# tud-amr/semantic_dsp_map

Measured on AMD Instinct MI355X. Metric: Mvoxels updated/sec (256^3 grid, 2M particles, VKITTI2 camera; whole hot-path frame), higher is better.
Workload: dtype f32

## Files before the change

### semantic_dsp_map_amd/csrc/kernels.hip

```cpp
#include <algorithm>

#include <type_traits>

#include <hip/hip_ext.h>
#include "sdm_internal.h"
#include "sdm_scratch.h"

#pragma clang fp contract(off)

namespace sdm {

namespace {

constexpr int TPB = 256;

#ifdef SDM_AB_TIMERS
}
__device__ unsigned long long g_dbg[6][8192 * 4];
namespace {
#define DBG_T() wall_clock64()
#define DBG_PUTK(k, i, v) do { if (blockIdx.x < 8192) g_dbg[k][blockIdx.x * 4 + (i)] = (unsigned long long)(v); } while (0)
#define DBG_PUT(i, v) DBG_PUTK(0, i, v)
#define DBG_LANE0(k, i) do { if (threadIdx.x == 0 && threadIdx.y == 0) DBG_PUTK(k, i, DBG_T()); } while (0)
#else
// ... 1497 lines not shown
      continue;
    }
    if (camz[i] > dpt * d.occl_coeff) continue;
    observed = true;
    vis[i] = true;
  }
  const uint32_t sub = (shard + (threadIdx.x & 63u)) & (ROW_SUBS - 1);
  uint32_t rq[S];
#pragma unroll
  for (int i = 1; i < S; ++i)
    if (vis[i]) {
      pib[i] = atomicAdd(&sc.bin_count[pixv[i]], 1u);
      rq[i] = atomicAdd(&sc.row_cnt[(size_t)(rowv[i] * ROW_SUBS + sub) * ROW_CNT_STRIDE], 1u);
    }
#pragma unroll
  for (int i = 1; i < S; ++i)
    if (vis[i]) {
      if (rq[i] < sc.row_cap && pib[i] < (1u << ROW_PIB_BITS)) {
        const uint32_t col = (uint32_t)(pixv[i] - rowv[i] * d.W);
        sc.row_list[(size_t)(rowv[i] * ROW_SUBS + sub) * sc.row_cap + rq[i]] =
            make_uint2((uint32_t)(((size_t)v << d.p_n) + i), col | pib[i] << ROW_COL_BITS);
      } else {
        sc.cnt->overflow = 1;
      }
    }
  if (dirty) rec_store_status<S>(rec, stv);
  if (dirty || wrote_free) st.vflag[lv] = VF_DIRTY;
  bool stamped = observed;
  if (!observed && valid_n == 0) stamped = im_ok && im_z <= im_depth;
  if (stamped) st.vts[lv] = (uint16_t)f.gts;
  if (dirty || wrote_free || stamped) mark_tile(st, lv, f.epoch);
}

constexpr int VIS_WORDS = 32;
constexpr int VIS_J = VIS_WORDS * 64 / TPB;

template <int S>
__global__ __launch_bounds__(TPB) void k_visibility(Dims d, State st, Scratch sc) {
  __shared__ unsigned long long wmask[VIS_WORDS];
  __shared__ uint32_t woff[VIS_WORDS + 1];
  __shared__ uint16_t full_list[VIS_WORDS * 64];
  __shared__ uint32_t n_full;
  DBG_LANE0(1, 0);
  const Frame f = sc.fa->f;
  const gptr<float> depth_img = as_global(sc.fa->depth);
  const uint32_t fgen = (uint32_t)sc.fa->force_generic, fcx = (uint32_t)sc.cnt->flood_complex;
  const bool generic = (fgen | fcx) != 0;
  if (blockIdx.x == 0 && threadIdx.x == 0) {
    sc.cnt->vis_flood_complex = fcx;
    sc.cnt->vis_flood_rounds = sc.cnt->flood_rounds;
    sc.cnt->vis_start_in_frustum = sc.cnt->start_in_frustum;
  }
  const int bx = f.bb1[0] - f.bb0[0], by = f.bb1[1] - f.bb0[1], bz = f.bb1[2] - f.bb0[2];
  if (bx <= 0 || by <= 0 || bz <= 0) return;
  const int wlo = f.bb0[0] >> 6, nwx = ((f.bb1[0] - 1) >> 6) - wlo + 1;
  const uint32_t n_words = (uint32_t)nwx * by * bz;
  for (uint32_t g0 = blockIdx.x * VIS_WORDS; g0 < n_words; g0 += gridDim.x * VIS_WORDS) {
  __syncthreads();
  if (threadIdx.x == 0) n_full = 0;
  if (threadIdx.x < VIS_WORDS) {
    const uint32_t g = g0 + threadIdx.x;
    unsigned long long m = 0;
    if (g < n_words) {
      const int wi = wlo + (int)(g % nwx);
      const int ay = f.bb0[1] + (int)((g / nwx) % by);
      const int az = f.bb0[2] + (int)(g / ((uint32_t)nwx * by));
      const uint32_t rz = axis_correct(az + f.eq[2], d.NZ);
      if (rz >= d.rz_begin && rz < d.rz_begin + d.rz_count) {
        const uint64_t *__restrict__ bits = generic ? sc.reach : sc.vmask;
        const int VY = d.NY + 1;
        unsigned long long w0[4], w1[4], lr[4];
        const int wi1 = wi + 1 < (int)sc.wpl ? wi + 1 : wi;
#pragma unroll
        for (int c = 0; c < 4; ++c) {
          const int y = ay + (c & 1), z = az + (c >> 1);
          const size_t lb = ((size_t)z * VY + y) * sc.wpl;
          lr[c] = sc.line_reach[(size_t)z * sc.wy + (y >> 6)];
          w0[c] = bits[lb + wi];
          w1[c] = bits[lb + wi1];
        }
        __builtin_amdgcn_sched_barrier(0);
#pragma unroll
        for (int c = 0; c < 4; ++c) {
          const int y = ay + (c & 1);
          const bool line_ok = generic || ((lr[c] >> (y & 63)) & 1ull);
          const unsigned long long w1m = wi + 1 < (int)sc.wpl ? w1[c] : 0ull;
          if (line_ok) m |= w0[c] | (w0[c] >> 1) | (w1m << 63);
        }
        const int x0 = wi << 6;
        const int lo = f.bb0[0] > x0 ? f.bb0[0] - x0 : 0;
        const int hi = f.bb1[0] - x0 < 64 ? f.bb1[0] - x0 : 64;
// ... 91 lines not shown
}

__device__ __forceinline__ void sift_down(uint32_t *a, uint32_t start, uint32_t end) {
  uint32_t root = start;
  while (2 * root + 1 <= end) {
    uint32_t child = 2 * root + 1, sw = root;
    if (a[sw] < a[child]) sw = child;
    if (child + 1 <= end && a[sw] < a[child + 1]) sw = child + 1;
    if (sw == root) return;
    uint32_t t = a[root];
    a[root] = a[sw];
    a[sw] = t;
    root = sw;
  }
}

constexpr int A7_ROWS = 16;
constexpr int A7_ITEMS = 16;
constexpr uint32_t CK_LIGHT_MAX = 4;
enum : uint8_t { CK_DONE = 0, CK_LIGHT = 1, CK_HEAVY = 2 };

__device__ __forceinline__ void ck_store(const Filter &flt, const Scratch &sc, float *__restrict__ ck_out, int finish, int p,
                                         const sdm_labeled_point &o, float ck) {
  if (finish) {
    const float ckk = ck * flt.p_detect + flt.noise_number;
    sc.ck_kappa[p] = ckk;
    sc.pix4[p] = make_float4(o.x, o.y, o.z, ckk);
    sc.pixt[p] = (uint32_t)o.track_id | (1u << 16);
  } else {
    ck_out[p] = ck;
  }
}

constexpr int BR_TPB = 640;
constexpr int BR_WAVES = BR_TPB / 64;
constexpr int BR_MAXW = 1 << ROW_COL_BITS;
template <int PPT>
__global__ __launch_bounds__(BR_TPB) __attribute__((amdgpu_waves_per_eu(PPT <= 4 ? 5 : 4, PPT <= 4 ? 5 : 4))) void k_bin_rows(Dims d, State st, Scratch sc) {
  static_assert(PPT == 2 || PPT == 4 || PPT * BR_TPB >= BR_MAXW, "eight pixels per thread cover the widest image");
  __shared__ uint32_t pre[BR_MAXW + 1];
  __shared__ uint32_t wave_tot[BR_WAVES];
  __shared__ uint32_t s_base;
  const int r = blockIdx.x;
  DBG_LANE0(2, 0);
  if (r == (int)gridDim.x - 1 && threadIdx.x < 64) alias_compact_wave(st);
  const bool overflow = sc.cnt->overflow != 0;
  const int lane = threadIdx.x & 63, wid = threadIdx.x >> 6;
  const int W = d.W;
  uint32_t c[PPT];
  const int j0 = PPT * (int)threadIdx.x;
#pragma unroll
  for (int u = 0; u < PPT; ++u) c[u] = (!overflow && j0 + u < W) ? sc.bin_count[r * W + j0 + u] : 0u;
  uint32_t sub_n = 0;
  if (threadIdx.x < ROW_SUBS && !overflow) {
    sub_n = sc.row_cnt[(size_t)(r * ROW_SUBS + threadIdx.x) * ROW_CNT_STRIDE];
    if (sub_n > sc.row_cap) sub_n = sc.row_cap;
  }
  uint32_t inc = 0;
#pragma unroll
  for (int u = 0; u < PPT; ++u) inc += c[u];
  const uint32_t mine = inc;
#pragma unroll
  for (int off = 1; off < 64; off <<= 1) {
    const uint32_t t = __shfl_up(inc, off, 64);
    if (lane >= off) inc += t;
  }
  if (lane == 63) wave_tot[wid] = inc;
  __syncthreads();
  uint32_t before = 0, total = 0;
#pragma unroll
  for (int w = 0; w < BR_WAVES; ++w) {
    if (w < wid) before += wave_tot[w];
    total += wave_tot[w];
  }
  {
    uint32_t run = before + inc - mine;
#pragma unroll
    for (int u = 0; u < PPT; ++u) {
      if (j0 + u < W) pre[j0 + u] = run;
      run += c[u];
    }
  }
  if (threadIdx.x == 0) {
    pre[W] = total;
    s_base = total ? atomicAdd(&sc.cnt->n_vis, total) : 0u;
    if (total && (s_base > sc.cap_vis || total > sc.cap_vis - s_base)) {
      sc.cnt->overflow = 1;
      pre[W] = 0;
    }
  }
  uint32_t sub_ex[ROW_SUBS + 1];
  {
    uint32_t run = 0;
#pragma unroll
    for (int k = 0; k < ROW_SUBS; ++k) {
      sub_ex[k] = run;
      run += (uint32_t)__shfl(sub_n, k, 64);
    }
    sub_ex[ROW_SUBS] = run;
  }
  __shared__ uint32_t s_sub[ROW_SUBS + 1];
  if (threadIdx.x == 0) {
#pragma unroll
    for (int k = 0; k <= ROW_SUBS; ++k) s_sub[k] = sub_ex[k];
  }
  __syncthreads();
  const uint32_t base = s_base;
  uint32_t *__restrict__ bs = sc.bin_start + (size_t)r * (W + 1);
  const bool row_over = total != 0 && pre[W] == 0;
  {
    const int h = d.window_half;
#pragma unroll
    for (int u = 0; u < PPT; ++u) {
      const int j = j0 + u;
      if (j < W) {
        const uint32_t n = row_over ? 0u : pre[j + h + 1 > W ? W : j + h + 1] - pre[j - h < 0 ? 0 : j - h];
        sc.row_win[r * W + j] = (uint8_t)(n > 255u ? 255u : n);
      }
    }
  }
  for (int j = threadIdx.x; j <= W; j += BR_TPB) bs[j] = row_over ? 0u : base + pre[j];
  if (total == 0 || row_over) {
    DBG_LANE0(2, 1);
    return;
  }
  const uint32_t n_row = s_sub[ROW_SUBS];
  for (uint32_t g = threadIdx.x; g < n_row; g += BR_TPB) {
    int sub = 0;
#pragma unroll
    for (int k = 1; k < ROW_SUBS; ++k) sub += s_sub[k] <= g ? 1 : 0;
    const uint2 e = sc.row_list[(size_t)(r * ROW_SUBS + sub) * sc.row_cap + (g - s_sub[sub])];
    sc.bin_idx[base + pre[e.y & (uint32_t)(BR_MAXW - 1)] + (e.y >> ROW_COL_BITS)] = e.x;
  }
  __syncthreads();
  const size_t slot_base = (size_t)d.v_begin << d.p_n;
#pragma unroll
  for (int u = 0; u < PPT; ++u) {
    const uint32_t n = c[u];
    if (!n) continue;
    const uint32_t p = (uint32_t)(r * W + j0 + u);
    const uint32_t s = base + pre[j0 + u];
    uint32_t *a = sc.bin_idx + s;
    auto small_bin = [&](auto kk) {
      constexpr int K = decltype(kk)::value;
      uint32_t v[K];
#pragma unroll
      for (int i = 0; i < K; ++i) v[i] = (uint32_t)i < n ? a[i] : 0xffffffffu;
#pragma unroll
      for (int pass = 0; pass < K; ++pass)
#pragma unroll
        for (int i = pass & 1; i + 1 < K; i += 2) {
          const uint32_t lo = v[i] < v[i + 1] ? v[i] : v[i + 1], hi = v[i] < v[i + 1] ? v[i + 1] : v[i];
          v[i] = lo;
// ... 36 lines not shown
    if (n > 1) {
      if (n <= 32) {
        for (uint32_t i = 1; i < n; ++i) {
          uint32_t x = a[i];
          uint32_t j = i;
          while (j > 0 && a[j - 1] > x) {
            a[j] = a[j - 1];
            --j;
          }
          a[j] = x;
        }
      } else {
        for (int start = (int)(n - 2) / 2; start >= 0; --start) sift_down(a, (uint32_t)start, n - 1);
        for (uint32_t end = n - 1; end > 0; --end) {
          uint32_t t = a[end];
          a[end] = a[0];
          a[0] = t;
          sift_down(a, 0, end - 1);
        }
      }
    }
    for (uint32_t i = 0; i < n; ++i) {
      const size_t li = (size_t)a[i] - slot_base;
      const float4 q = st.pos4[li];
      const SlotRef sr = slot_ref_li(st, d.p_n, li);
      sc.vp4[s + i] = make_float4(q.x, q.y, q.z, sr.w());
      sc.vtf[s + i] = (uint32_t)sr.track() | ((uint32_t)st.forget[li] << 16);
      sc.vpix[s + i] = p;
    }
  }
  DBG_LANE0(2, 1);
}

__global__ __launch_bounds__(TPB) void k_ck_classify(Dims d, Filter flt, Scratch sc, float *__restrict__ ck_out, int finish) {
  const uint32_t p = blockIdx.x * blockDim.x + threadIdx.x;
  const int W = d.W, H = d.H, h = d.window_half;
  const bool in_image = p < (uint32_t)(W * H);
  const bool overflow = sc.cnt->overflow != 0;
  sdm_labeled_point o;
  o.is_valid = 0;
  uint32_t total = 0;
  if (in_image) {
    o = load_point(sc.fa->cloud, p);
    const int i = (int)p / W;
    uint32_t rw[A7_ROWS];
#pragma unroll
    for (int r = 0; r < A7_ROWS; ++r) {
      const int ni = i + r - h;
      const bool ok = r <= 2 * h && ni >= 0 && ni < H;
      rw[r] = sc.row_win[(int)p + (ok ? (r - h) * W : 0)];
    }
    __builtin_amdgcn_sched_barrier(0);
#pragma unroll
    for (int r = 0; r < A7_ROWS; ++r) {
      const int ni = i + r - h;
      total += (r <= 2 * h && ni >= 0 && ni < H) ? rw[r] : 0u;
    }
  }
  uint8_t cls = CK_DONE;
  if (in_image && o.is_valid && total != 0 && !overflow) cls = total <= CK_LIGHT_MAX ? CK_LIGHT : CK_HEAVY;
  const unsigned long long hm = __ballot(cls == CK_HEAVY);
  if (hm) {
    const uint32_t lane = threadIdx.x & 63u;
    const uint32_t shard = blockIdx.x & (VIS_SHARDS - 1);
    uint32_t base = 0;
    if (lane == 0) base = atomicAdd(&sc.cnt->shard[shard].heavy, (uint32_t)__popcll(hm));
    base = (uint32_t)__shfl((int)base, 0, 64);
    if (cls == CK_HEAVY) sc.ck_heavy[shard * sc.cap_heavy + base + (uint32_t)__popcll(hm & ((1ull << lane) - 1ull))] = p;
  }
  if (!in_image) return;
  if (!finish) {
    sc.pix4[p] = make_float4(o.x, o.y, o.z, 0.f);
    sc.pixt[p] = o.is_valid ? ((uint32_t)o.track_id | (1u << 16)) : 0u;
  }
  if (!o.is_valid) {
    if (finish) sc.pixt[p] = 0;
  } else if (cls == CK_DONE) {
    ck_store(flt, sc, ck_out, finish, (int)p, o, 0.f);
  }
  sc.ck_class[p] = cls;
}


template <bool FAST>
__device__ __forceinline__ float ck_term(const Filter &flt, const float *__restrict__ pdf, const float4 pv, const uint32_t tf,
                                         const sdm_labeled_point &o, float rsig, bool &skip) {
  const uint16_t ptrack = (uint16_t)(tf & 0xffffu);
  skip = flt.independent && ptrack != o.track_id;
  const float fg = flt.forget[(tf >> 16) & 7];
  float gk = query_pdf_r<FAST>(pdf, pv.x, o.x, o.sigma, rsig) * query_pdf_r<FAST>(pdf, pv.y, o.y, o.sigma, rsig) *
             query_pdf_r<FAST>(pdf, pv.z, o.z, o.sigma, rsig);
  if (!flt.independent) {
    gk *= fg;
    if (ptrack != o.track_id) gk *= flt.id_transition;
  }
  return pv.w * gk;
}

__device__ __forceinline__ void ck_light_pixel(const Dims &d, const Filter &flt, const State &st, const Scratch &sc,
                                               float *__restrict__ ck_out, int finish, int p) {
  const bool mine = p < d.W * d.H && sc.ck_class[p] == CK_LIGHT;
  sdm_labeled_point o;
  uint32_t ss[A7_ROWS], ee[A7_ROWS];
  if (mine) {
    o = load_point(sc.fa->cloud, p);
    const int h = d.window_half;
    const int i = p / d.W, j = p - i * d.W;
    const int j0 = j - h < 0 ? 0 : j - h;
    const int j1 = j + h >= d.W ? d.W - 1 : j + h;
#pragma unroll
    for (int r = 0; r < A7_ROWS; ++r) {
      const int ni = i + r - h;
      ss[r] = ee[r] = 0;
      if (r <= 2 * h && ni >= 0 && ni < d.H) {
        ss[r] = sc.bin_start[ni * (d.W + 1) + j0];
// ... 30 lines not shown
#endif
constexpr uint32_t CK_TERM_CAP = SDM_CK_TERM_CAP;

#ifndef SDM_CK_HEAVY_PER_LIST
#define SDM_CK_HEAVY_PER_LIST 28
#endif
constexpr uint32_t CK_HEAVY_BLOCKS = SDM_CK_HEAVY_PER_LIST * VIS_SHARDS;
#ifndef SDM_CK_WAVES
#define SDM_CK_WAVES 7
#endif
#define CK_WAVES_ATTR __attribute__((amdgpu_waves_per_eu(SDM_CK_WAVES, SDM_CK_WAVES)))

__global__ __launch_bounds__(A7_ROWS *A7_ITEMS) CK_WAVES_ATTR void k_ck(Dims d, Filter flt, State st, Scratch sc,
                                                          float *__restrict__ ck_out, int finish) {
  DBG_LANE0(3, 0);
  if (blockIdx.x >= CK_HEAVY_BLOCKS) {
    ck_light_pixel(d, flt, st, sc, ck_out, finish,
                   (int)((blockIdx.x - CK_HEAVY_BLOCKS) * (A7_ROWS * A7_ITEMS) + threadIdx.y * A7_ROWS + threadIdx.x));
    DBG_LANE0(3, 1);
    return;
  }
  __shared__ float rowsum[A7_ITEMS][A7_ROWS];
  __shared__ uint32_t rowoff[A7_ITEMS * A7_ROWS + 1];
  __shared__ uint32_t rowbeg[A7_ITEMS * A7_ROWS];
  __shared__ float opx[A7_ITEMS][5];
  __shared__ uint32_t otrk[A7_ITEMS];
  __shared__ float term[CK_TERM_CAP];
  __shared__ uint8_t rowof[CK_TERM_CAP];
  const int r = threadIdx.x, it = threadIdx.y;
  const int lane = it * A7_ROWS + r;
  const int h = d.window_half;
  const uint32_t shard = blockIdx.x & (VIS_SHARDS - 1);
  const uint32_t n = sc.cnt->shard[shard].heavy;
  const float *__restrict__ pdf = st.pdf;
  const gptr<sdm_labeled_point> cloud_img = as_global(sc.fa->cloud);
  __shared__ uint32_t s_q0, s_slow;
  for (;;) {
    __syncthreads();
    if (lane == 0) {
      s_q0 = atomicAdd(&sc.cnt->shard[shard].heavy_ticket, (uint32_t)A7_ITEMS);
      s_slow = 0;
    }
    __syncthreads();
    const uint32_t q0 = s_q0;
    if (q0 >= n) break;
#ifdef SDM_AB_TIMERS
    if (lane == 0) g_dbg[3][blockIdx.x * 4 + 2] += 1;
#endif
    const uint32_t q = q0 + it;
    int p = 0;
    uint32_t s = 0, e = 0;
    sdm_labeled_point o;
    if (q < n) {
      p = (int)sc.ck_heavy[shard * sc.cap_heavy + q];
      o = load_point(sc.fa->cloud, p);
      const int i = p / d.W, j = p - i * d.W;
      const int ni = i + r - h;
      if (r <= 2 * h && ni >= 0 && ni < d.H) {
        const int j0 = j - h < 0 ? 0 : j - h;
        const int j1 = j + h >= d.W ? d.W - 1 : j + h;
        s = sc.bin_start[ni * (d.W + 1) + j0];
        e = sc.bin_start[ni * (d.W + 1) + j1 + 1];
      }
      if (r == 0) {
        opx[it][0] = o.x;
        opx[it][1] = o.y;
// ... 1159 lines not shown
    const uint32_t seg = n_tiles <= TPB * OCC_SEG_MAX ? ((n_tiles + TPB - 1) / TPB + 15u) / 16u * 16u : 0u;
    if (seg) grid = dim3(std::min<uint32_t>(OCC_GRID, n_tiles));
    SDM_DISPATCH_S(k_occupancy, grid, s, d, flt.occ_threshold, st, cnt, fa, n_tiles, seg);
  }
}


void launch_set_frame(FrameArgs *fa_dev, const FrameArgs &fa, hipStream_t s) {
  hipLaunchKernelGGL(k_set_frame, dim3(1), dim3(TPB), 0, s, fa_dev, fa);
}
const void *set_frame_kernel() { return reinterpret_cast<const void *>(k_set_frame); }

void launch_frustum(const Dims &d, const Scratch &sc, hipStream_t s) {
  static bool lds_attr_set = false;
  if (!lds_attr_set) {
    (void)hipFuncSetAttribute(reinterpret_cast<const void *>(k_flood2d), hipFuncAttributeMaxDynamicSharedMemorySize, 152 * 1024);
    lds_attr_set = true;
  }
  const size_t max_words = (size_t)(d.NY + 1) * (d.NZ + 1) * sc.wpl;
  const unsigned g_mask = (unsigned)std::min<size_t>(blocks_for(max_words * 64), 4096);
  const unsigned g_line = (unsigned)std::min<size_t>(blocks_for((size_t)sc.wy * (d.NZ + 1) * 64), 256);
  hipLaunchKernelGGL(k_vertex_mask, dim3(g_mask), dim3(TPB), 0, s, d, sc.fa_side, sc.vmask, sc.wpl, sc.cnt);
  hipLaunchKernelGGL(k_line_info, dim3(g_line), dim3(TPB), 0, s, d, sc.fa_side, sc.vmask, sc.wpl, sc.wy, sc.line_ne, sc.line_ey, sc.line_ez,
                     sc.cnt);
  hipLaunchKernelGGL(k_flood2d, dim3(1), dim3(TPB), (size_t)(d.NZ + 1) * sc.wy * 8 * 4, s, d, sc.fa_side, sc.vmask, sc.wpl, sc.wy, sc.line_ey,
                     sc.line_ez, sc.line_reach, sc.cnt);
  hipLaunchKernelGGL(k_flood_generic, dim3(1), dim3(1024), 0, s, d, sc.fa_side, sc.vmask, sc.reach, sc.wpl, sc.cnt);
}

void launch_visibility(const Dims &d, const Filter &flt, const State &st, const Scratch &sc, float *ck_out, int finish, hipStream_t s,
                       hipEvent_t vis_done) {
  {
    const size_t max_words = (size_t)((d.NX + 63) / 64 + 1) * d.NY * d.NZ;
    dim3 grid((unsigned)std::min<size_t>(blocks_for(max_words, VIS_WORDS), 2048));
    if (vis_done) {
      switch (d.p_n) {
        case 1: hipExtLaunchKernelGGL(k_visibility<2>, grid, dim3(TPB), 0, s, nullptr, vis_done, 0, d, st, sc); break;
        case 2: hipExtLaunchKernelGGL(k_visibility<4>, grid, dim3(TPB), 0, s, nullptr, vis_done, 0, d, st, sc); break;
        case 3: hipExtLaunchKernelGGL(k_visibility<8>, grid, dim3(TPB), 0, s, nullptr, vis_done, 0, d, st, sc); break;
        default: hipExtLaunchKernelGGL(k_visibility<16>, grid, dim3(TPB), 0, s, nullptr, vis_done, 0, d, st, sc); break;
      }
    } else {
      SDM_DISPATCH_S(k_visibility, grid, s, d, st, sc);
    }
  }
  if (d.W <= 2 * BR_TPB) hipLaunchKernelGGL(k_bin_rows<2>, dim3((unsigned)d.H), dim3(BR_TPB), 0, s, d, st, sc);
  else if (d.W <= 4 * BR_TPB) hipLaunchKernelGGL(k_bin_rows<4>, dim3((unsigned)d.H), dim3(BR_TPB), 0, s, d, st, sc);
  else hipLaunchKernelGGL(k_bin_rows<8>, dim3((unsigned)d.H), dim3(BR_TPB), 0, s, d, st, sc);
  hipLaunchKernelGGL(k_ck_classify, dim3(blocks_for((size_t)d.W * d.H)), dim3(TPB), 0, s, d, flt, sc, ck_out, finish);
}

void launch_ck(const Dims &d, const Filter &flt, const State &st, const Scratch &sc, float *ck_out, int finish, hipStream_t s) {
  hipLaunchKernelGGL(k_ck, dim3(CK_HEAVY_BLOCKS + blocks_for((size_t)d.W * d.H, A7_ROWS * A7_ITEMS)), dim3(A7_ROWS, A7_ITEMS), 0, s, d, flt, st, sc,
                     ck_out, finish);
}
void launch_ck_finish(const Dims &d, const Filter &flt, const Scratch &sc, const float *parts, int n_parts, size_t part_stride, hipStream_t s) {
  hipLaunchKernelGGL(k_ck_finish, dim3(blocks_for((size_t)d.W * d.H)), dim3(TPB), 0, s, d, flt, sc, parts, n_parts,
                     part_stride ? part_stride : (size_t)d.W * d.H);
}
void launch_ck_reduce_chunk(const float *stage, const float *own_part, float *full, uint32_t chunk, int world, int rank, hipStream_t s) {
  hipLaunchKernelGGL(k_ck_reduce_chunk, dim3((chunk + TPB - 1) / TPB), dim3(TPB), 0, s, stage, own_part, full, chunk, world, rank);
}
void launch_weight(const Dims &d, const Filter &flt, const State &st, const Scratch &sc, hipStream_t s, const float *ck_raw) {
  const int side = 2 * d.window_half + 1;
#define SDM_WEIGHT(UU, RR)                                                                                              \
  if (ck_raw) hipLaunchKernelGGL((k_weight<UU, RR, true>), dim3(WT_GRID), dim3(64 * WT_WAVES), 0, s, d, flt, st, sc, ck_raw); \
  else hipLaunchKernelGGL((k_weight<UU, RR, false>), dim3(WT_GRID), dim3(64 * WT_WAVES), 0, s, d, flt, st, sc, ck_raw);
  if (side * side <= 64) {
    SDM_WEIGHT(4, 1)
  } else if (side * side <= 128) {
    SDM_WEIGHT(4, 2)
  } else {
    SDM_WEIGHT(2, 4)
  }
#undef SDM_WEIGHT
}

int launch_birth_prepare(const Dims &d, const Filter &flt, const BirthOrder &bo, const State &st,
                         const Scratch &sc, hipStream_t s) {
  const size_t hw = (size_t)d.W * d.H;
  const size_t total = hw * flt.nb;
  if (flt.use_rng) {
// ... 189 lines not shown
```

### semantic_dsp_map_amd/csrc/lifecycle.hip

```cpp
#include <rocrand/rocrand.h>

#include <chrono>
#include <cmath>
#include <cstdlib>
#include <mutex>

#include "sdm_map.h"

#pragma clang fp contract(off)

namespace {

thread_local std::string g_last_error;

__attribute__((constructor(101))) void sdm_runtime_defaults() {
  setenv("HIP_FORCE_DEV_KERNARG", "1", 0);
}

constexpr double GRAPH_PIECES_US = 110.0, GRAPH_CHAIN_US = 170.0;
constexpr int LAUNCHES_PER_FRAME = 50;

__global__ void k_noop() {}

}
// ... 410 lines not shown
  A(m->st.alias, 2 + 2 * ALIAS_CAP);
  m->st.alias_cap = ALIAS_CAP;
  HIP_TRY(hipMemsetAsync(m->st.alias, 0, 8, m->stream));
  A(m->st.alias_filter, ALIAS_FILTER_WORDS);
  HIP_TRY(hipMemsetAsync(m->st.alias_filter, 0, ALIAS_FILTER_WORDS * 4, m->stream));
  A(m->st.res, d.v_count);
  A(m->st.stamps_x, d.NX);
  A(m->st.stamps_y, d.NY);
  A(m->st.stamps_z, d.NZ);
  A(m->st.pdf, PDF_NUM);
  m->noise_n = 1000000;
  A(m->st.noise, m->noise_n);
  HIP_TRY(hipMemsetAsync(m->st.noise, 0, (size_t)m->noise_n * 4, m->stream));
  {
    std::vector<float> pdf;
    build_pdf_table(pdf);
    HIP_TRY(hipMemcpyAsync(m->st.pdf, pdf.data(), PDF_NUM * 4, hipMemcpyHostToDevice, m->stream));
    HIP_TRY(hipStreamSynchronize(m->stream));
  }
  Scratch &sc = m->sc;
  sc.wpl = (int)((d.NX + 1 + 63) / 64);
  const size_t n_words = (size_t)(d.NZ + 1) * (d.NY + 1) * sc.wpl;
  A(sc.vmask, n_words);
  A(sc.reach, n_words);
  sc.wy = (int)((d.NY + 1 + 63) / 64);
  const size_t n_line_words = (size_t)(d.NZ + 1) * sc.wy;
  A(sc.line_ne, n_line_words);
  A(sc.line_ey, n_line_words);
  A(sc.line_ez, n_line_words);
  A(sc.line_reach, n_line_words);
  A(m->d_depth, hw);
  A(m->d_cloud, hw);
  A(sc.bin_count, hw + 1 + (size_t)d.H * ROW_SUBS * ROW_CNT_STRIDE);
  A(sc.row_win, hw);
  sc.row_cnt = sc.bin_count + hw + 1;
  A(sc.bin_start, (size_t)d.H * (d.W + 1));
  size_t cap_vis = cfg->max_visible > 0 ? (size_t)cfg->max_visible
                                        : std::min<size_t>(n_slots + (size_t)VIS_SHARDS * 256 * d.S, (size_t)16 << 20);
  cap_vis = (cap_vis + VIS_SHARDS - 1) / VIS_SHARDS * VIS_SHARDS;
  cap_vis = std::min<size_t>(cap_vis, 0xffffff00u);
  sc.cap_vis = (uint32_t)cap_vis;
  {
    const size_t row_total = std::min<size_t>(cap_vis, std::max<size_t>(2 * cap_vis / (size_t)d.H, (size_t)2 * d.W * d.S));
    sc.row_cap = (uint32_t)std::max<size_t>(64, (row_total + row_total / 4) / ROW_SUBS + 64);
  }
  A(sc.row_list, (size_t)d.H * ROW_SUBS * sc.row_cap);
  A(sc.bin_idx, cap_vis);
  A(sc.vpix, cap_vis);
  A(sc.vp4, cap_vis);
  A(sc.vtf, cap_vis);
  A(sc.pix4, hw);
  A(sc.pixt, hw);
  A(sc.ck_kappa, hw);
  sc.cap_heavy = (uint32_t)(((hw + 255) / 256 + VIS_SHARDS - 1) / VIS_SHARDS * 256);
  A(sc.ck_heavy, (size_t)sc.cap_heavy * VIS_SHARDS);
  A(sc.ck_class, hw);
  m->ck_chunk = (uint32_t)(((hw + shard_count - 1) / shard_count + 63) / 64 * 64);
  A(m->d_ck_part, (size_t)m->ck_chunk * shard_count);
  for (auto &r : m->raw) {
    A(r.depth, hw);
    A(r.static_mask, hw);
    A(r.label_to_inst, 256);
    A(r.bbox, 6 * MAX_CLOUD_OBJECTS);
  }
  A(sc.b_valid, hw + 1);
  A(sc.b_rank, hw + 1);
  sc.cap_move = (uint32_t)std::min<size_t>((size_t)d.V * d.S, (size_t)1 << 18);
  A(m->d_counts_local, HALO_OBJ);
  const size_t mv_cnt_n = move_count_elems();
  A(sc.mv_cnt, mv_cnt_n);
  A(sc.mv_list, 8192);
  A(sc.mv_nlist, 4);
  HIP_TRY(hipMemsetAsync(sc.mv_nlist, 0, 4 * sizeof(uint32_t), m->stream));
  A(sc.mv_nmem, 8192);
  A(sc.mv_mem, move_member_elems(n_slots));
  A(sc.mv_tot, move_total_elems());
  HIP_TRY(hipMemsetAsync(sc.mv_tot, 0, move_total_elems() * sizeof(uint32_t), m->stream));
  A(m->d_track_bits, 2048);
  A(sc.mv_copy, sc.cap_move);
  A(sc.track_to_obj, 65536);
  HIP_TRY(hipMemsetAsync(sc.track_to_obj, 0xFF, 65536, m->stream));
  size_t scan_need = scan_scratch_elems(hw + 1);
  A(sc.scan_scratch, scan_need + 16);
  A(sc.scan_scratch_b, scan_scratch_elems(hw + 1) + 16);
  HIP_TRY(hipMemsetAsync(sc.scan_scratch, 0, (scan_need + 16) * 4, m->stream));
  HIP_TRY(hipMemsetAsync(sc.scan_scratch_b, 0, (scan_scratch_elems(hw + 1) + 16) * 4, m->stream));
  A(sc.mv_row, (size_t)d.v_count * MV_ROW);
// ... 203 lines not shown
```

### semantic_dsp_map_amd/csrc/sdm_internal.h

```cpp
#pragma once
#include <hip/hip_runtime.h>
#include <stdint.h>

#include "../../include/sdm.h"

#pragma clang fp contract(off)

namespace sdm {

constexpr uint32_t INVALID_INDEX = 0xffffffffu;
constexpr uint16_t OWNER_NONE = 0xFFFF;
constexpr int PDF_NUM = 20000;
#define SDM_OCC_INIT_WEIGHT 0.05f
#define SDM_MIN_RIGHT_PDF 0.1f

enum : uint8_t { ST_INVALID = 0, ST_UPDATED = 1, ST_REGULAR_BORN = 2, ST_GUESSED_BORN = 3, ST_COPIED = 4, ST_TIMEPTC = 5 };

struct Dims {
  int x_n, y_n, z_n, p_n;
  uint32_t NX, NY, NZ, S;
  uint32_t V;
  uint32_t v_begin;
  uint32_t v_count;
  uint32_t rz_begin, rz_count;
// ... 24 lines not shown
  float forget[8];
  int independent;
  int consider_depth_noise;
  int nb;
  int use_rng;
  int noise_n;
};

struct Counters {
  uint32_t n_vis;
  uint32_t n_birth_success;
  uint32_t n_birth_attempts;
  uint32_t n_resampled;
  uint32_t n_moved;
  uint32_t n_move_reinserted;
  uint32_t n_frustum_voxels;
  uint32_t n_occupied;
  uint32_t n_free;
  uint32_t overflow;
  uint32_t n_valid_px;
  uint32_t n_halo_dropped;
  uint32_t vis_flood_complex, vis_flood_rounds, vis_start_in_frustum;
  uint32_t n_moved_b[2];
  uint32_t pad[2];
  struct alignas(128) ShardLine {
    uint32_t vis;
    uint32_t fv;
    uint32_t heavy;
    uint32_t birth;
    uint32_t resample;
    uint32_t sweep;
    uint32_t sweep_tiles;
    uint32_t heavy_ticket;
    uint32_t pad[24];
  };
  ShardLine shard[64];
  uint32_t flood_complex;
  uint32_t flood_rounds;
  uint32_t start_in_frustum;
  uint32_t flood_pad[29];
};
static_assert(sizeof(Counters::ShardLine) == 128, "one cache line per shard");
constexpr uint32_t VIS_SHARDS = 64;
constexpr uint32_t ROW_SUBS = 8;
constexpr int ROW_COL_BITS = 12, ROW_PIB_BITS = 32 - ROW_COL_BITS;
constexpr uint32_t ROW_CNT_STRIDE = 32;
constexpr uint32_t OWNER_CHUNK = 4096;
constexpr uint32_t OWNER_GROUP = 64;
__host__ __device__ constexpr size_t owner_flag_bytes(size_t n_slots) {
  return ((n_slots + OWNER_CHUNK - 1) / OWNER_CHUNK + OWNER_GROUP - 1) / OWNER_GROUP * OWNER_GROUP;
}
__host__ __device__ constexpr size_t owner_flag2_bytes(size_t n_slots) { return (owner_flag_bytes(n_slots) / OWNER_GROUP + 4095) / 4096 * 4096; }
constexpr int MAX_STAMP_UPDATES = 96;
struct StampUpdates {
  int n;
  uint32_t value;
  uint16_t entry[MAX_STAMP_UPDATES];
};
struct Cursors {
  int32_t birth_cursor;
  int32_t move_cursor;
  uint32_t move_list_overflow;
};

constexpr size_t REC_BYTES_PER_SLOT = 10;
__host__ __device__ constexpr uint32_t rec_bytes(uint32_t S) { return (uint32_t)REC_BYTES_PER_SLOT * (S - 1u); }
__host__ __device__ constexpr size_t rec_array_bytes(size_t v_count, uint32_t S) { return (v_count + 64) * rec_bytes(S) + 64; }
typedef float rec_f32 __attribute__((aligned(2)));
typedef uint32_t rec_v4u __attribute__((ext_vector_type(4), aligned(2)));
typedef uint32_t rec_v2u __attribute__((ext_vector_type(2), aligned(2)));

struct SlotRef {
  unsigned char *r;
  uint32_t L, k;
  __host__ __device__ __forceinline__ float w() const { return *reinterpret_cast<const rec_f32 *>(r + 4u * k); }
  __host__ __device__ __forceinline__ uint16_t ts() const { return *reinterpret_cast<const uint16_t *>(r + 4u * L + 2u * k); }
  __host__ __device__ __forceinline__ uint16_t track() const { return *reinterpret_cast<const uint16_t *>(r + 6u * L + 2u * k); }
  __host__ __device__ __forceinline__ uint8_t label() const { return r[8u * L + k]; }
// ... 373 lines not shown
```

### semantic_dsp_map_amd/csrc/sdm_scratch.h

```cpp
#pragma once
#include "sdm_internal.h"

namespace sdm {

struct BirthOrder {
  int off[10];
  int cols[9];
};

struct MoveCopy {
  float x, y, z;
  uint32_t forget_bits;
  float w;
  uint16_t ts, track, owner;
  uint8_t label, status;
  uint32_t voxel;
};
static_assert(sizeof(MoveCopy) == 32, "MoveCopy layout");

constexpr int MAX_MOVE_OBJECTS = 48;
constexpr int MAX_REMOVE_TRACKS = 128;
constexpr int HALO_OBJ = 64;
constexpr int HALO_RECORD_BYTES = 36;
constexpr int HALO_HEADER_BYTES = 16;
// ... 2 lines not shown
  int n;
  float T[MAX_MOVE_OBJECTS][12];
  uint16_t track[MAX_MOVE_OBJECTS];
};

struct FrameArgs {
  Frame f;
  StampUpdates su;
  MoveSet ms;
  int n_obj;
  int n_remove;
  uint32_t mv_seq;
  uint32_t mv_batch;
  int force_generic;
  const float *depth;
  const sdm_labeled_point *cloud;
  uint16_t remove[MAX_REMOVE_TRACKS];
};
static_assert(sizeof(FrameArgs) <= 3400, "FrameArgs travels as a kernel argument (4 KB limit, with the launch's other arguments)");

constexpr int MV_ROW = 16;
constexpr int MV_DIRECT = MV_ROW - 2;
constexpr uint32_t MV_FIRST = 0x100u;
struct Scratch {
  const FrameArgs *fa = nullptr;
  const FrameArgs *fa_side = nullptr;
  const FrameArgs *fa_moves = nullptr;
  uint64_t *vmask = nullptr, *reach = nullptr;
  int wpl = 0;
  uint64_t *line_ne = nullptr, *line_ey = nullptr, *line_ez = nullptr, *line_reach = nullptr;
  int wy = 0;
  uint32_t *bin_count = nullptr, *bin_start = nullptr;
  uint32_t *row_cnt = nullptr;
  uint8_t *row_win = nullptr;
  uint2 *row_list = nullptr;
  uint32_t row_cap = 0;
  uint32_t cap_vis = 0;
  uint32_t *bin_idx = nullptr, *vpix = nullptr;
  float4 *vp4 = nullptr;
  uint32_t *vtf = nullptr;
  float4 *pix4 = nullptr;
  uint32_t *pixt = nullptr;
  float *ck_kappa = nullptr;
  uint8_t *ck_class = nullptr;
  uint32_t *ck_heavy = nullptr;
  uint32_t cap_heavy = 0;
  uint32_t *b_valid = nullptr, *b_rank = nullptr;
  uint32_t *bkey_a = nullptr, *bval_a = nullptr, *bkey_b = nullptr, *bval_b = nullptr;
  float4 *bpos = nullptr;
  uint32_t *mv_cnt = nullptr;
  uint32_t *mv_list = nullptr, *mv_nlist = nullptr;
  uint32_t *mv_nmem = nullptr, *mv_mem = nullptr, *mv_tot = nullptr;
  MoveCopy *mv_copy = nullptr;
  uint32_t cap_move = 0;
  unsigned char *halo_send = nullptr;
  const unsigned char *halo_recv = nullptr;
  uint32_t halo_cap = 0;
  uint32_t halo_world = 1;
  uint8_t *track_to_obj = nullptr;
  uint32_t *scan_scratch = nullptr, *sort_scratch = nullptr;
  uint32_t *scan_scratch_b = nullptr;
  uint32_t *mv_row = nullptr, *mv_next = nullptr;
  Counters *cnt = nullptr;
  Cursors *cur = nullptr;
};

constexpr int MAX_CLOUD_OBJECTS = 64;
// ... 102 lines not shown
```

Before: 95820.

## Fuse pixel classification into row binning and add ticketed visibility chunks

Removes the separate k_ck_classify kernel and its row_win byte buffer. k_bin_rows now sums bin counts over the vertical window directly, runs an extra row scan to classify each pixel as done, light or heavy, and writes the heavy list with per-wave shard assignment. The visibility kernel also gets atomic per-shard ticket-based dynamic chunk scheduling instead of a static grid-stride loop. This saves one launch and the row_win round trip, but each bin_rows block now reads up to 2h+1 rows of bin_count and does an extra scan. Heavy-list capacity is recomputed with a host-side overrun check.

```diff
diff --git a/semantic_dsp_map_amd/csrc/kernels.hip b/semantic_dsp_map_amd/csrc/kernels.hip
--- a/semantic_dsp_map_amd/csrc/kernels.hip
+++ b/semantic_dsp_map_amd/csrc/kernels.hip
@@ -1553,7 +1553,17 @@
   if (dirty || wrote_free || stamped) mark_tile(st, lv, f.epoch);
 }
 
-constexpr int VIS_WORDS = 32;
+#ifndef SDM_VIS_TICKETS
+#define SDM_VIS_TICKETS 1
+#endif
+#ifndef SDM_VIS_WORDS
+#define SDM_VIS_WORDS 32
+#endif
+constexpr int VIS_WORDS = SDM_VIS_WORDS;
+#ifndef SDM_VIS_GRID
+#define SDM_VIS_GRID 2048
+#endif
+static_assert(VIS_WORDS == 16 || VIS_WORDS == 32 || VIS_WORDS == 64, "one wave scans the words' popcounts; whole candidates per thread");
 constexpr int VIS_J = VIS_WORDS * 64 / TPB;
 
 template <int S>
@@ -1576,8 +1586,26 @@
   if (bx <= 0 || by <= 0 || bz <= 0) return;
   const int wlo = f.bb0[0] >> 6, nwx = ((f.bb1[0] - 1) >> 6) - wlo + 1;
   const uint32_t n_words = (uint32_t)nwx * by * bz;
+#if SDM_VIS_TICKETS
+  __shared__ uint32_t s_ticket;
+  const uint32_t n_chunks = (n_words + VIS_WORDS - 1) / VIS_WORDS;
+  const uint32_t tshard = blockIdx.x & (VIS_SHARDS - 1);
+  const uint32_t tfirst = gridDim.x + ((tshard - gridDim.x) & (VIS_SHARDS - 1));
+  uint32_t chunk = blockIdx.x;
+  for (bool first = true;; first = false) {
+  __syncthreads();
+  if (!first) {
+    if (tfirst >= n_chunks) break;
+    if (threadIdx.x == 0) s_ticket = tfirst + VIS_SHARDS * atomicAdd(&sc.cnt->shard[tshard].vis_ticket, 1u);
+    __syncthreads();
+    chunk = s_ticket;
+  }
+  if (chunk >= n_chunks) break;
+  const uint32_t g0 = chunk * VIS_WORDS;
+#else
   for (uint32_t g0 = blockIdx.x * VIS_WORDS; g0 < n_words; g0 += gridDim.x * VIS_WORDS) {
   __syncthreads();
+#endif
   if (threadIdx.x == 0) n_full = 0;
   if (threadIdx.x < VIS_WORDS) {
     const uint32_t g = g0 + threadIdx.x;
@@ -1735,12 +1763,12 @@
   }
 }
 
-constexpr int BR_TPB = 640;
-constexpr int BR_WAVES = BR_TPB / 64;
 constexpr int BR_MAXW = 1 << ROW_COL_BITS;
 template <int PPT>
-__global__ __launch_bounds__(BR_TPB) __attribute__((amdgpu_waves_per_eu(PPT <= 4 ? 5 : 4, PPT <= 4 ? 5 : 4))) void k_bin_rows(Dims d, State st, Scratch sc) {
+__global__ __launch_bounds__(BR_TPB) __attribute__((amdgpu_waves_per_eu(PPT <= 4 ? 5 : 4, PPT <= 4 ? 5 : 4))) void k_bin_rows(
+    Dims d, Filter flt, State st, Scratch sc, float *__restrict__ ck_out, int finish) {
   static_assert(PPT == 2 || PPT == 4 || PPT * BR_TPB >= BR_MAXW, "eight pixels per thread cover the widest image");
+  static_assert(PPT == br_ppt(PPT == 2 ? 2 * BR_TPB : PPT == 4 ? 4 * BR_TPB : BR_MAXW - 1), "the launch picks PPT by br_ppt");
   __shared__ uint32_t pre[BR_MAXW + 1];
   __shared__ uint32_t wave_tot[BR_WAVES];
   __shared__ uint32_t s_base;
@@ -1749,7 +1777,7 @@
   if (r == (int)gridDim.x - 1 && threadIdx.x < 64) alias_compact_wave(st);
   const bool overflow = sc.cnt->overflow != 0;
   const int lane = threadIdx.x & 63, wid = threadIdx.x >> 6;
-  const int W = d.W;
+  const int W = d.W, H = d.H, h = d.window_half;
   uint32_t c[PPT];
   const int j0 = PPT * (int)threadIdx.x;
 #pragma unroll
@@ -1759,33 +1787,114 @@
     sub_n = sc.row_cnt[(size_t)(r * ROW_SUBS + threadIdx.x) * ROW_CNT_STRIDE];
     if (sub_n > sc.row_cap) sub_n = sc.row_cap;
   }
-  uint32_t inc = 0;
-#pragma unroll
-  for (int u = 0; u < PPT; ++u) inc += c[u];
-  const uint32_t mine = inc;
-#pragma unroll
-  for (int off = 1; off < 64; off <<= 1) {
-    const uint32_t t = __shfl_up(inc, off, 64);
-    if (lane >= off) inc += t;
-  }
-  if (lane == 63) wave_tot[wid] = inc;
-  __syncthreads();
-  uint32_t before = 0, total = 0;
-#pragma unroll
-  for (int w = 0; w < BR_WAVES; ++w) {
-    if (w < wid) before += wave_tot[w];
-    total += wave_tot[w];
-  }
-  {
+  sdm_labeled_point o[PPT];
+  uint32_t cw[PPT];
+  int jc[PPT];
+#pragma unroll
+  for (int u = 0; u < PPT; ++u) {
+    jc[u] = j0 + u < W ? j0 + u : W - 1;
+    o[u] = load_point(sc.fa->cloud, (size_t)(r * W + jc[u]));
+    cw[u] = 0;
+  }
+  constexpr int RB = 32 / PPT < A7_ROWS ? 32 / PPT : A7_ROWS;
+#pragma unroll
+  for (int k0 = 0; k0 < A7_ROWS; k0 += RB) {
+    if (k0 > 2 * h) break;
+    uint32_t t[RB][PPT];
+#pragma unroll
+    for (int k = 0; k < RB; ++k) {
+      const int ni = r + k0 + k - h;
+      const int row = (k0 + k <= 2 * h && ni >= 0 && ni < H) ? ni : r;
+#pragma unroll
+      for (int u = 0; u < PPT; ++u) t[k][u] = sc.bin_count[row * W + jc[u]];
+    }
+    __builtin_amdgcn_sched_barrier(0);
+#pragma unroll
+    for (int k = 0; k < RB; ++k) {
+      const int ni = r + k0 + k - h;
+      const bool ok = k0 + k <= 2 * h && ni >= 0 && ni < H;
+#pragma unroll
+      for (int u = 0; u < PPT; ++u) cw[u] += ok ? t[k][u] : 0u;
+    }
+  }
+#pragma unroll
+  for (int u = 0; u < PPT; ++u)
+    if (overflow || j0 + u >= W) cw[u] = 0;
+  auto row_scan = [&](const uint32_t(&v)[PPT]) {
+    uint32_t inc = 0;
+#pragma unroll
+    for (int u = 0; u < PPT; ++u) inc += v[u];
+    const uint32_t mine = inc;
+#pragma unroll
+    for (int off = 1; off < 64; off <<= 1) {
+      const uint32_t t = __shfl_up(inc, off, 64);
+      if (lane >= off) inc += t;
+    }
+    if (lane == 63) wave_tot[wid] = inc;
+    __syncthreads();
+    uint32_t before = 0, total = 0;
+#pragma unroll
+    for (int w = 0; w < BR_WAVES; ++w) {
+      if (w < wid) before += wave_tot[w];
+      total += wave_tot[w];
+    }
     uint32_t run = before + inc - mine;
 #pragma unroll
     for (int u = 0; u < PPT; ++u) {
       if (j0 + u < W) pre[j0 + u] = run;
-      run += c[u];
-    }
-  }
+      run += v[u];
+    }
+    if (threadIdx.x == 0) pre[W] = total;
+    return total;
+  };
+  row_scan(cw);
+  __syncthreads();
+  {
+    uint8_t cls[PPT];
+    unsigned long long hm[PPT];
+    uint32_t nh = 0;
+#pragma unroll
+    for (int u = 0; u < PPT; ++u) {
+      const int j = j0 + u;
+      cls[u] = CK_DONE;
+      if (j < W) {
+        const uint32_t n = pre[j + h + 1 > W ? W : j + h + 1] - pre[j - h < 0 ? 0 : j - h];
+        if (o[u].is_valid && n != 0) cls[u] = n <= CK_LIGHT_MAX ? CK_LIGHT : CK_HEAVY;
+      }
+      hm[u] = __ballot(cls[u] == CK_HEAVY);
+      nh += (uint32_t)__popcll(hm[u]);
+    }
+    if (nh) {
+      const uint32_t shard = heavy_shard_of((uint32_t)r, (uint32_t)wid);
+      uint32_t at = 0;
+      if (lane == 0) at = atomicAdd(&sc.cnt->shard[shard].heavy, nh);
+      at = (uint32_t)__shfl((int)at, 0, 64);
+#pragma unroll
+      for (int u = 0; u < PPT; ++u) {
+        if (cls[u] == CK_HEAVY)
+          sc.ck_heavy[shard * sc.cap_heavy + at + (uint32_t)__popcll(hm[u] & ((1ull << lane) - 1ull))] = (uint32_t)(r * W + j0 + u);
+        at += (uint32_t)__popcll(hm[u]);
+      }
+    }
+#pragma unroll
+    for (int u = 0; u < PPT; ++u) {
+      if (j0 + u >= W) continue;
+      const int p = r * W + j0 + u;
+      if (!finish) {
+        sc.pix4[p] = make_float4(o[u].x, o[u].y, o[u].z, 0.f);
+        sc.pixt[p] = o[u].is_valid ? ((uint32_t)o[u].track_id | (1u << 16)) : 0u;
+      }
+      if (!o[u].is_valid) {
+        if (finish) sc.pixt[p] = 0;
+      } else if (cls[u] == CK_DONE) {
+        ck_store(flt, sc, ck_out, finish, p, o[u], 0.f);
+      }
+      sc.ck_class[p] = cls[u];
+    }
+  }
+  __syncthreads();
+  const uint32_t total = row_scan(c);
   if (threadIdx.x == 0) {
-    pre[W] = total;
     s_base = total ? atomicAdd(&sc.cnt->n_vis, total) : 0u;
     if (total && (s_base > sc.cap_vis || total > sc.cap_vis - s_base)) {
       sc.cnt->overflow = 1;
@@ -1811,17 +1920,6 @@
   const uint32_t base = s_base;
   uint32_t *__restrict__ bs = sc.bin_start + (size_t)r * (W + 1);
   const bool row_over = total != 0 && pre[W] == 0;
-  {
-    const int h = d.window_half;
-#pragma unroll
-    for (int u = 0; u < PPT; ++u) {
-      const int j = j0 + u;
-      if (j < W) {
-        const uint32_t n = row_over ? 0u : pre[j + h + 1 > W ? W : j + h + 1] - pre[j - h < 0 ? 0 : j - h];
-        sc.row_win[r * W + j] = (uint8_t)(n > 255u ? 255u : n);
-      }
-    }
-  }
   for (int j = threadIdx.x; j <= W; j += BR_TPB) bs[j] = row_over ? 0u : base + pre[j];
   if (total == 0 || row_over) {
     DBG_LANE0(2, 1);
@@ -1924,55 +2022,6 @@
   DBG_LANE0(2, 1);
 }
 
-__global__ __launch_bounds__(TPB) void k_ck_classify(Dims d, Filter flt, Scratch sc, float *__restrict__ ck_out, int finish) {
-  const uint32_t p = blockIdx.x * blockDim.x + threadIdx.x;
-  const int W = d.W, H = d.H, h = d.window_half;
-  const bool in_image = p < (uint32_t)(W * H);
-  const bool overflow = sc.cnt->overflow != 0;
-  sdm_labeled_point o;
-  o.is_valid = 0;
-  uint32_t total = 0;
-  if (in_image) {
-    o = load_point(sc.fa->cloud, p);
-    const int i = (int)p / W;
-    uint32_t rw[A7_ROWS];
-#pragma unroll
-    for (int r = 0; r < A7_ROWS; ++r) {
-      const int ni = i + r - h;
-      const bool ok = r <= 2 * h && ni >= 0 && ni < H;
-      rw[r] = sc.row_win[(int)p + (ok ? (r - h) * W : 0)];
-    }
-    __builtin_amdgcn_sched_barrier(0);
-#pragma unroll
-    for (int r = 0; r < A7_ROWS; ++r) {
-      const int ni = i + r - h;
-      total += (r <= 2 * h && ni >= 0 && ni < H) ? rw[r] : 0u;
-    }
-  }
-  uint8_t cls = CK_DONE;
-  if (in_image && o.is_valid && total != 0 && !overflow) cls = total <= CK_LIGHT_MAX ? CK_LIGHT : CK_HEAVY;
-  const unsigned long long hm = __ballot(cls == CK_HEAVY);
-  if (hm) {
-    const uint32_t lane = threadIdx.x & 63u;
-    const uint32_t shard = blockIdx.x & (VIS_SHARDS - 1);
-    uint32_t base = 0;
-    if (lane == 0) base = atomicAdd(&sc.cnt->shard[shard].heavy, (uint32_t)__popcll(hm));
-    base = (uint32_t)__shfl((int)base, 0, 64);
-    if (cls == CK_HEAVY) sc.ck_heavy[shard * sc.cap_heavy + base + (uint32_t)__popcll(hm & ((1ull << lane) - 1ull))] = p;
-  }
-  if (!in_image) return;
-  if (!finish) {
-    sc.pix4[p] = make_float4(o.x, o.y, o.z, 0.f);
-    sc.pixt[p] = o.is_valid ? ((uint32_t)o.track_id | (1u << 16)) : 0u;
-  }
-  if (!o.is_valid) {
-    if (finish) sc.pixt[p] = 0;
-  } else if (cls == CK_DONE) {
-    ck_store(flt, sc, ck_out, finish, (int)p, o, 0.f);
-  }
-  sc.ck_class[p] = cls;
-}
-
 
 template <bool FAST>
 __device__ __forceinline__ float ck_term(const Filter &flt, const float *__restrict__ pdf, const float4 pv, const uint32_t tf,
@@ -2069,6 +2118,9 @@
   const int h = d.window_half;
   const uint32_t shard = blockIdx.x & (VIS_SHARDS - 1);
   const uint32_t n = sc.cnt->shard[shard].heavy;
+#ifdef SDM_AB_TIMERS
+  if (threadIdx.x == 0 && threadIdx.y == 0) g_dbg[3][blockIdx.x * 4 + 3] = n;
+#endif
   const float *__restrict__ pdf = st.pdf;
   const gptr<sdm_labeled_point> cloud_img = as_global(sc.fa->cloud);
   __shared__ uint32_t s_q0, s_slow;
@@ -3294,7 +3346,7 @@
                        hipEvent_t vis_done) {
   {
     const size_t max_words = (size_t)((d.NX + 63) / 64 + 1) * d.NY * d.NZ;
-    dim3 grid((unsigned)std::min<size_t>(blocks_for(max_words, VIS_WORDS), 2048));
+    dim3 grid((unsigned)std::min<size_t>(blocks_for(max_words, VIS_WORDS), SDM_VIS_GRID));
     if (vis_done) {
       switch (d.p_n) {
         case 1: hipExtLaunchKernelGGL(k_visibility<2>, grid, dim3(TPB), 0, s, nullptr, vis_done, 0, d, st, sc); break;
@@ -3306,10 +3358,11 @@
       SDM_DISPATCH_S(k_visibility, grid, s, d, st, sc);
     }
   }
-  if (d.W <= 2 * BR_TPB) hipLaunchKernelGGL(k_bin_rows<2>, dim3((unsigned)d.H), dim3(BR_TPB), 0, s, d, st, sc);
-  else if (d.W <= 4 * BR_TPB) hipLaunchKernelGGL(k_bin_rows<4>, dim3((unsigned)d.H), dim3(BR_TPB), 0, s, d, st, sc);
-  else hipLaunchKernelGGL(k_bin_rows<8>, dim3((unsigned)d.H), dim3(BR_TPB), 0, s, d, st, sc);
-  hipLaunchKernelGGL(k_ck_classify, dim3(blocks_for((size_t)d.W * d.H)), dim3(TPB), 0, s, d, flt, sc, ck_out, finish);
+  switch (br_ppt(d.W)) {
+    case 2: hipLaunchKernelGGL(k_bin_rows<2>, dim3((unsigned)d.H), dim3(BR_TPB), 0, s, d, flt, st, sc, ck_out, finish); break;
+    case 4: hipLaunchKernelGGL(k_bin_rows<4>, dim3((unsigned)d.H), dim3(BR_TPB), 0, s, d, flt, st, sc, ck_out, finish); break;
+    default: hipLaunchKernelGGL(k_bin_rows<8>, dim3((unsigned)d.H), dim3(BR_TPB), 0, s, d, flt, st, sc, ck_out, finish); break;
+  }
 }
 
 void launch_ck(const Dims &d, const Filter &flt, const State &st, const Scratch &sc, float *ck_out, int finish, hipStream_t s) {
diff --git a/semantic_dsp_map_amd/csrc/lifecycle.hip b/semantic_dsp_map_amd/csrc/lifecycle.hip
--- a/semantic_dsp_map_amd/csrc/lifecycle.hip
+++ b/semantic_dsp_map_amd/csrc/lifecycle.hip
@@ -466,7 +466,6 @@
   A(m->d_depth, hw);
   A(m->d_cloud, hw);
   A(sc.bin_count, hw + 1 + (size_t)d.H * ROW_SUBS * ROW_CNT_STRIDE);
-  A(sc.row_win, hw);
   sc.row_cnt = sc.bin_count + hw + 1;
   A(sc.bin_start, (size_t)d.H * (d.W + 1));
   size_t cap_vis = cfg->max_visible > 0 ? (size_t)cfg->max_visible
@@ -486,7 +485,17 @@
   A(sc.pix4, hw);
   A(sc.pixt, hw);
   A(sc.ck_kappa, hw);
-  sc.cap_heavy = (uint32_t)(((hw + 255) / 256 + VIS_SHARDS - 1) / VIS_SHARDS * 256);
+  sc.cap_heavy = heavy_list_cap(d.H, d.W);
+  {
+    std::vector<uint32_t> listed(VIS_SHARDS, 0);
+    const int per_wave = 64 * br_ppt(d.W);
+    for (int r = 0; r < d.H; ++r)
+      for (int w = 0; w * per_wave < d.W; ++w) listed[heavy_shard_of((uint32_t)r, (uint32_t)w)] += (uint32_t)std::min(per_wave, d.W - w * per_wave);
+    if (*std::max_element(listed.begin(), listed.end()) > sc.cap_heavy || BR_WAVES * per_wave < d.W) {
+      set_error("sdm_create", __FILE__, __LINE__, "a heavy-pixel list of the weight update can overrun its capacity");
+      return SDM_ERR_INVALID_ARGUMENT;
+    }
+  }
   A(sc.ck_heavy, (size_t)sc.cap_heavy * VIS_SHARDS);
   A(sc.ck_class, hw);
   m->ck_chunk = (uint32_t)(((hw + shard_count - 1) / shard_count + 63) / 64 * 64);
diff --git a/semantic_dsp_map_amd/csrc/sdm_internal.h b/semantic_dsp_map_amd/csrc/sdm_internal.h
--- a/semantic_dsp_map_amd/csrc/sdm_internal.h
+++ b/semantic_dsp_map_amd/csrc/sdm_internal.h
@@ -80,7 +80,8 @@
     uint32_t sweep;
     uint32_t sweep_tiles;
     uint32_t heavy_ticket;
-    uint32_t pad[24];
+    uint32_t vis_ticket;
+    uint32_t pad[23];
   };
   ShardLine shard[64];
   uint32_t flood_complex;
@@ -92,6 +93,13 @@
 constexpr uint32_t VIS_SHARDS = 64;
 constexpr uint32_t ROW_SUBS = 8;
 constexpr int ROW_COL_BITS = 12, ROW_PIB_BITS = 32 - ROW_COL_BITS;
+constexpr int BR_TPB = 640;
+constexpr int BR_WAVES = BR_TPB / 64;
+__host__ __device__ constexpr int br_ppt(int W) { return W <= 2 * BR_TPB ? 2 : W <= 4 * BR_TPB ? 4 : 8; }
+__host__ __device__ constexpr uint32_t heavy_shard_of(uint32_t row, uint32_t wave) { return (row * BR_WAVES + wave) & (VIS_SHARDS - 1); }
+__host__ __device__ constexpr uint32_t heavy_list_cap(int H, int W) {
+  return ((uint32_t)H * BR_WAVES + VIS_SHARDS - 1) / VIS_SHARDS * 64u * (uint32_t)br_ppt(W);
+}
 constexpr uint32_t ROW_CNT_STRIDE = 32;
 constexpr uint32_t OWNER_CHUNK = 4096;
 constexpr uint32_t OWNER_GROUP = 64;
diff --git a/semantic_dsp_map_amd/csrc/sdm_scratch.h b/semantic_dsp_map_amd/csrc/sdm_scratch.h
--- a/semantic_dsp_map_amd/csrc/sdm_scratch.h
+++ b/semantic_dsp_map_amd/csrc/sdm_scratch.h
@@ -58,7 +58,6 @@
   int wy = 0;
   uint32_t *bin_count = nullptr, *bin_start = nullptr;
   uint32_t *row_cnt = nullptr;
-  uint8_t *row_win = nullptr;
   uint2 *row_list = nullptr;
   uint32_t row_cap = 0;
   uint32_t cap_vis = 0;
```

Measured after the change: 93810. 2.1% lower.
